# dylkot/cNMF

Measured on NVIDIA H100. Metric: NMF restarts/sec on NxG counts, K-sweep x100 seeds, 1/2/4/8 H100 vs sklearn CPU, higher is better.
Workload: dtype f32 (2-pass split-fp16 tensor-core products of group-normalised factors x exact integer counts, fp32 accumulate)

## Files before the change

### cnmf_b200/csrc/nmf_kernels.cu

```cuda
#include "nmf_kernels.cuh"

#include <cuda_fp16.h>

namespace cnmf {

namespace {

constexpr float EPSILON_F32 = 1.1920928955078125e-07f;

template <typename T>
__device__ __forceinline__ T block_sum(T v, T* smem ) {
  const int lane = threadIdx.x & 31, warp = threadIdx.x >> 5;
  v = warp_sum(v);
  __syncthreads();
  if (lane == 0) smem[warp] = v;
  __syncthreads();
  const int nw = (blockDim.x + 31) >> 5;
  T r = (threadIdx.x < nw) ? smem[threadIdx.x] : T(0);
  if (warp == 0) r = warp_sum(r);
  return r;
}

__global__ void split_tf32_kernel(const float* __restrict__ src, float* __restrict__ hi, float* __restrict__ lo,
                                  long long n4) {
// ... 227 lines not shown

template <int KP, int VEC>
__device__ __forceinline__ void load_items(const float* __restrict__ pF, const float* __restrict__ pN, int nsplit,
                                           long long sstride, int K, unsigned ld, int n_left,
                                           float2 (&fv)[KP][VecIO<VEC>::NP], float2 (&nv)[KP][VecIO<VEC>::NP]) {
  constexpr int NP = VecIO<VEC>::NP;
#pragma unroll
  for (int i = 0; i < KP; ++i) {
    if (i < K) {
      const unsigned off = (unsigned)i * ld;
      VecIO<VEC>::ld(pF + off, fv[i]);
      VecIO<VEC>::ld(pN + off, nv[i]);
    } else {
#pragma unroll
      for (int p = 0; p < NP; ++p) {
        fv[i][p] = make_float2(0.f, 0.f);
        nv[i][p] = make_float2(0.f, 0.f);
      }
    }
  }
  if (nsplit > 1) {
    for (int s = 1; s < nsplit; ++s) {
      const float* pS = pN + s * sstride;
#pragma unroll
      for (int i = 0; i < KP; ++i) {
        if (i < K) {
          float2 t[NP];
          VecIO<VEC>::ld(pS + (unsigned)i * ld, t);
#pragma unroll
          for (int p = 0; p < NP; ++p) nv[i][p] = add2(nv[i][p], t[p]);
        }
      }
    }
  }
  if (n_left < VEC) {
#pragma unroll
    for (int i = 0; i < KP; ++i)
#pragma unroll
      for (int p = 0; p < NP; ++p) {
        if (2 * p >= n_left) { nv[i][p].x = 0.f; fv[i][p].x = 0.f; }
        if (2 * p + 1 >= n_left) { nv[i][p].y = 0.f; fv[i][p].y = 0.f; }
      }
  }
}

template <int VEC>
__device__ __forceinline__ void store_items(float* pF, float* pH, float* pL, unsigned off,
                                            const float2 (&v)[VecIO<VEC>::NP], const float2 (&pscale)[VecIO<VEC>::NP]) {
  constexpr int NP = VecIO<VEC>::NP;
  VecIO<VEC>::st(pF + off, v);
  if (pH) {
    float2 h[NP], l[NP];
#pragma unroll
    for (int p = 0; p < NP; ++p) {
      const float2 sv = mul2(v[p], pscale[p]);
      h[p] = make_float2(to_tf32(sv.x), to_tf32(sv.y));
      const float2 rest = add2(sv, neg2(h[p]));
      l[p] = make_float2(to_tf32(rest.x), to_tf32(rest.y));
    }
    VecIO<VEC>::st(pH + off, h);
    VecIO<VEC>::st(pL + off, l);
  }
}

template <int KP> struct FusedGramCfg {
  static constexpr int WARPS = UPD_THREADS / 32;
  static constexpr int TPC = KP <= 4 ? 1 : (KP <= 8 ? 2 : 4);
  static constexpr int RB = KP / TPC;
  static constexpr int NG = WARPS / TPC;
  static constexpr int VALS = RB * KP;
  static constexpr int STRIDE = (VALS / 4) % 2 ? VALS : VALS + 4;
};

template <int KP, int TILE>
__device__ __forceinline__ void fused_gram_tile(float* tile, double* gsum) {
  using C = FusedGramCfg<KP>;
  const int lane = threadIdx.x & 31, warp = threadIdx.x >> 5;
  const int rb = warp % C::TPC, grp = warp / C::TPC;
  float2 acc[C::RB][KP];
#pragma unroll
  for (int a = 0; a < C::RB; ++a)
#pragma unroll
    for (int i = 0; i < KP; ++i) acc[a][i] = make_float2(0.f, 0.f);
  const float4* t4 = reinterpret_cast<const float4*>(tile);
  constexpr int QUADS = TILE / 4, ROW4 = TILE / 4;
#pragma unroll 1
  for (int q = grp * 32 + lane; q < QUADS; q += 32 * C::NG) {
    float4 v[KP], va[C::RB];
#pragma unroll
    for (int i = 0; i < KP; ++i) v[i] = t4[i * ROW4 + q];
#pragma unroll
    for (int a = 0; a < C::RB; ++a) va[a] = t4[(rb * C::RB + a) * ROW4 + q];
#pragma unroll
    for (int a = 0; a < C::RB; ++a)
#pragma unroll
      for (int i = 0; i < KP; ++i) {
        acc[a][i] = fma2(make_float2(va[a].x, va[a].y), make_float2(v[i].x, v[i].y), acc[a][i]);
        acc[a][i] = fma2(make_float2(va[a].z, va[a].w), make_float2(v[i].z, v[i].w), acc[a][i]);
      }
  }
  __syncthreads();
  float* scratch = tile + threadIdx.x * C::STRIDE;
#pragma unroll
  for (int a = 0; a < C::RB; ++a)
#pragma unroll
    for (int i4 = 0; i4 < KP / 4; ++i4) {
      float4 q;
      q.x = acc[a][4 * i4 + 0].x + acc[a][4 * i4 + 0].y;
      q.y = acc[a][4 * i4 + 1].x + acc[a][4 * i4 + 1].y;
      q.z = acc[a][4 * i4 + 2].x + acc[a][4 * i4 + 2].y;
      q.w = acc[a][4 * i4 + 3].x + acc[a][4 * i4 + 3].y;
      *reinterpret_cast<float4*>(scratch + a * KP + 4 * i4) = q;
    }
  __syncthreads();
  for (int e = threadIdx.x; e < KP * KP; e += UPD_THREADS) {
    const int row = e / KP, i = e % KP;
    const int erb = row / C::RB, a = row % C::RB;
    double sum = 0.0;
#pragma unroll
    for (int g = 0; g < C::NG; ++g) {
      const float* src = tile + (size_t)((erb + C::TPC * g) * 32) * C::STRIDE + a * KP + i;
#pragma unroll 8
      for (int l = 0; l < 32; ++l) sum += (double)src[l * C::STRIDE];
    }
    gsum[e] += sum;
  }
  __syncthreads();
}

struct SymGramMap {
  static __device__ __forceinline__ void owner(int bi, int bj, int& warp, int& slot) {
    const int id = bi * 4 + bj - (bi * (bi + 1)) / 2;
    warp = id / 3;
    slot = id % 3;
  }
};

template <int KP, int TILE, int W>
__device__ __forceinline__ void sym_gram_accumulate(const float* tile, float2 (&acc)[3][KP / 4][KP / 4]) {
  constexpr int RB = KP / 4;
  constexpr int NB = W == 3 ? 1 : 3;
  constexpr int BI[3] = {W == 0 ? 0 : (W == 1 ? 0 : (W == 2 ? 1 : 3)), W == 0 ? 0 : (W == 1 ? 1 : 2), W == 0 ? 0 : (W == 1 ? 1 : 2)};
  constexpr int BJ[3] = {W == 0 ? 0 : (W == 1 ? 3 : (W == 2 ? 3 : 3)), W == 0 ? 1 : (W == 1 ? 1 : 2), W == 0 ? 2 : (W == 1 ? 2 : 3)};
  const int lane = threadIdx.x & 31;
  const float4* t4 = reinterpret_cast<const float4*>(tile);
  constexpr int QUADS = TILE / 4, ROW4 = TILE / 4;
#pragma unroll 1
  for (int q = lane; q < QUADS; q += 32) {
    float4 v[4][RB];
#pragma unroll
    for (int blk = 0; blk < 4; ++blk) {
      bool used = false;
#pragma unroll
      for (int k = 0; k < NB; ++k) used = used || BI[k] == blk || BJ[k] == blk;
      if (used) {
#pragma unroll
        for (int a = 0; a < RB; ++a) v[blk][a] = t4[(blk * RB + a) * ROW4 + q];
      }
    }
#pragma unroll
    for (int k = 0; k < NB; ++k)
#pragma unroll
      for (int a = 0; a < RB; ++a)
#pragma unroll
        for (int b = 0; b < RB; ++b) {
          const float4 x = v[BI[k]][a], y = v[BJ[k]][b];
          acc[k][a][b] = fma2(make_float2(x.x, x.y), make_float2(y.x, y.y), acc[k][a][b]);
          acc[k][a][b] = fma2(make_float2(x.z, x.w), make_float2(y.z, y.w), acc[k][a][b]);
        }
  }
}

template <int KP> struct SymGramPlan {
  static constexpr int NUP = KP * (KP + 1) / 2;
  static constexpr int ROUNDS = (NUP + UPD_THREADS - 1) / UPD_THREADS;
};
constexpr int SYM_PLAN_WORDS = 3 * 2 * UPD_THREADS;

template <int KP>
__device__ __forceinline__ void sym_gram_plan(int* plan) {
  constexpr int RB = KP / 4;
  constexpr int STRIDE = 3 * RB * RB + 1;
  static_assert(SymGramPlan<KP>::ROUNDS <= 2, "plan buffer holds two rounds");
#pragma unroll
  for (int r = 0; r < SymGramPlan<KP>::ROUNDS; ++r) {
    const int t = threadIdx.x + r * UPD_THREADS;
    int row = 0, rem = t;
    while (row < KP - 1 && rem >= KP - row) { rem -= KP - row; ++row; }
    const int i = row + rem;
    int src = -1, e1 = 0, e2 = 0;
    if (t < SymGramPlan<KP>::NUP) {
      int w, slot;
      SymGramMap::owner(row / RB, i / RB, w, slot);
      src = (w * 32) * STRIDE + (slot * RB + row % RB) * RB + i % RB;
      e1 = row * KP + i;
      e2 = i * KP + row;
    }
    plan[(r * 3 + 0) * UPD_THREADS + threadIdx.x] = src;
    plan[(r * 3 + 1) * UPD_THREADS + threadIdx.x] = e1;
    plan[(r * 3 + 2) * UPD_THREADS + threadIdx.x] = e2;
  }
}

template <int KP, int TILE>
__device__ __forceinline__ void fused_gram_tile_sym(float* tile, double* gsum, const int* plan) {
  constexpr int RB = KP / 4;
  constexpr int STRIDE = 3 * RB * RB + 1;
  static_assert(UPD_THREADS == 128, "four warps share the ten blocks");
  static_assert(UPD_THREADS * STRIDE <= KP * TILE, "reduction scratch must fit in the tile it aliases");
  const int warp = threadIdx.x >> 5;
  float2 acc[3][RB][RB];
#pragma unroll
  for (int k = 0; k < 3; ++k)
#pragma unroll
    for (int a = 0; a < RB; ++a)
#pragma unroll
      for (int b = 0; b < RB; ++b) acc[k][a][b] = make_float2(0.f, 0.f);
  switch (warp) {
    case 0: sym_gram_accumulate<KP, TILE, 0>(tile, acc); break;
    case 1: sym_gram_accumulate<KP, TILE, 1>(tile, acc); break;
    case 2: sym_gram_accumulate<KP, TILE, 2>(tile, acc); break;
    default: sym_gram_accumulate<KP, TILE, 3>(tile, acc); break;
  }
  __syncthreads();
  float* scratch = tile + threadIdx.x * STRIDE;
#pragma unroll
  for (int k = 0; k < 3; ++k)
#pragma unroll
    for (int a = 0; a < RB; ++a)
#pragma unroll
      for (int b = 0; b < RB; ++b) scratch[(k * RB + a) * RB + b] = acc[k][a][b].x + acc[k][a][b].y;
  __syncthreads();
#pragma unroll
  for (int r = 0; r < SymGramPlan<KP>::ROUNDS; ++r) {
    const int so = plan[(r * 3 + 0) * UPD_THREADS + threadIdx.x];
    if (so >= 0) {
      const int e1 = plan[(r * 3 + 1) * UPD_THREADS + threadIdx.x], e2 = plan[(r * 3 + 2) * UPD_THREADS + threadIdx.x];
      const float* src = tile + so;
      double sum = 0.0;
#pragma unroll 8
      for (int l = 0; l < 32; ++l) sum += (double)src[l * STRIDE];
      gsum[e1] += sum;
      if (e2 != e1) gsum[e2] += sum;
    }
  }
  __syncthreads();
}

template <int TILE>
__device__ __forceinline__ void emit_tile_f16(const FactorView& f, const float* tile, int K, int o, int t0) {
  static_assert(TILE == 512, "one lane owns four 16-byte groups of a 512-column tile");
  const int lane = threadIdx.x & 31, warp = threadIdx.x >> 5;
  float4 ps[4];
#pragma unroll
  for (int j = 0; j < 4; ++j) {
    const int col = t0 + 4 * lane + 128 * j;
    ps[j] = make_float4(1.f, 1.f, 1.f, 1.f);
    if (f.piece_scale && col < f.ld) ps[j] = *reinterpret_cast<const float4*>(f.piece_scale + col);
  }
  const int group = t0 / TILE;
  for (int c = warp; c < K; c += UPD_THREADS / 32) {
    const float4* src = reinterpret_cast<const float4*>(tile + c * TILE);
    float2 v[4][2];
    float m = 0.f;
#pragma unroll
    for (int j = 0; j < 4; ++j) {
      const float4 q = src[lane + 32 * j];
      v[j][0] = mul2(make_float2(q.x, q.y), make_float2(ps[j].x, ps[j].y));
      v[j][1] = mul2(make_float2(q.z, q.w), make_float2(ps[j].z, ps[j].w));
      m = fmaxf(fmaxf(m, fmaxf(v[j][0].x, v[j][0].y)), fmaxf(v[j][1].x, v[j][1].y));
    }
#pragma unroll
    for (int s = 16; s > 0; s >>= 1) m = fmaxf(m, __shfl_xor_sync(0xffffffffu, m, s));
    const float sc = f16_group_scale(m);
    const float2 inv = bcast2(__uint_as_float(0x7f000000u - __float_as_uint(sc)));
    const long long rowoff = (long long)(o + c) * f.ld;
    if (lane == 0) f.tile_scale[(long long)(o + c) * f.n_ktiles + group] = sc;
    __half* ph = static_cast<__half*>(f.P_hi) + rowoff + t0 + 4 * lane;
    __half* pm = static_cast<__half*>(f.P_mid) + rowoff + t0 + 4 * lane;
    const int cols_left = f.ld - (t0 + 4 * lane);
#pragma unroll
    for (int j = 0; j < 4; ++j) {
      if (128 * j < cols_left) {
        const float2 x01 = mul2(v[j][0], inv), x23 = mul2(v[j][1], inv);
        const __half2 h01 = __float22half2_rn(x01), h23 = __float22half2_rn(x23);
        const float2 r01 = add2(x01, neg2(__half22float2(h01))), r23 = add2(x23, neg2(__half22float2(h23)));
        const __half2 m01 = __float22half2_rn(r01), m23 = __float22half2_rn(r23);
        uint2 oh, om;
        oh.x = *reinterpret_cast<const uint32_t*>(&h01); oh.y = *reinterpret_cast<const uint32_t*>(&h23);
        om.x = *reinterpret_cast<const uint32_t*>(&m01); om.y = *reinterpret_cast<const uint32_t*>(&m23);
        *reinterpret_cast<uint2*>(ph + 128 * j) = oh;
        *reinterpret_cast<uint2*>(pm + 128 * j) = om;
      }
    }
  }
}

__device__ __forceinline__ float4 lds128(unsigned addr) {
  float4 v;
  asm("ld.shared.v4.f32 {%0, %1, %2, %3}, [%4];" : "=f"(v.x), "=f"(v.y), "=f"(v.z), "=f"(v.w) : "r"(addr));
  return v;
}

template <int KP, int VEC, bool GRAM, bool RAGGED, bool SIMPLE>
__device__ __forceinline__ float2 mu_components(float* __restrict__ pFc, float* pH, float* pL, const float* __restrict__ pNc,
                                                int nsplit, long long sstride, unsigned ld, unsigned g_row, int K, float l1,
                                                float l2, int n_left, const float2 (&fv)[KP][VecIO<VEC>::NP],
                                                const float2 (&pscale)[VecIO<VEC>::NP], float* myF) {
  constexpr int NP = VecIO<VEC>::NP;
  constexpr int TILE = UPD_THREADS * VEC;
  float2 sacc = make_float2(0.f, 0.f);
  float2 nvn[NP], nvn2[NP];
  VecIO<VEC>::ld(pNc, nvn);
  VecIO<VEC>::ld(pNc + (1 < K ? ld : 0u), nvn2);
#pragma unroll 3
  for (int c = 0; c < K; ++c) {
    float2 den[NP];
#pragma unroll
    for (int i4 = 0; i4 < KP / 4; ++i4) {
      const float4 gq = lds128(g_row + 16 * i4);
#pragma unroll
      for (int p = 0; p < NP; ++p) {
        den[p] = i4 == 0 ? mul2(bcast2(gq.x), fv[0][p]) : fma2(bcast2(gq.x), fv[4 * i4 + 0][p], den[p]);
        den[p] = fma2(bcast2(gq.y), fv[4 * i4 + 1][p], den[p]);
        den[p] = fma2(bcast2(gq.z), fv[4 * i4 + 2][p], den[p]);
        den[p] = fma2(bcast2(gq.w), fv[4 * i4 + 3][p], den[p]);
      }
    }
    g_row += 4 * KP;
    float2 fvc[NP], nvc[NP], out[NP];
    VecIO<VEC>::ld(myF, fvc);
#pragma unroll
    for (int p = 0; p < NP; ++p) { nvc[p] = nvn[p]; nvn[p] = nvn2[p]; }
    VecIO<VEC>::ld(pNc + ((c + 2 < K) ? 2u * ld : 0u), nvn2);
    if constexpr (!SIMPLE) {
      for (int s = 1; s < nsplit; ++s) {
        float2 t[NP];
        VecIO<VEC>::ld(pNc + s * sstride, t);
#pragma unroll
        for (int p = 0; p < NP; ++p) nvc[p] = add2(nvc[p], t[p]);
      }
    }
    if constexpr (RAGGED) {
#pragma unroll
      for (int p = 0; p < NP; ++p) {
        if (2 * p >= n_left) nvc[p].x = 0.f;
        if (2 * p + 1 >= n_left) nvc[p].y = 0.f;
      }
    }
#pragma unroll
    for (int p = 0; p < NP; ++p) {
      float2 d = fma2(bcast2(l2), fvc[p], add2(den[p], bcast2(l1)));
      d.x = (d.x < FLT_MIN_NORMAL) ? EPSILON_F32 : d.x;
      d.y = (d.y < FLT_MIN_NORMAL) ? EPSILON_F32 : d.y;
      out[p] = mul2(fvc[p], div_nr2(nvc[p], d));
      sacc = fma2(nvc[p], out[p], sacc);
    }
    if constexpr (SIMPLE) {
      VecIO<VEC>::st(pFc, out);
    } else {
      store_items<VEC>(pFc, pH, pL, 0u, out, pscale);
      if (pH) { pH += ld; pL += ld; }
    }
    if constexpr (GRAM) VecIO<VEC>::st(myF, out);
    pFc += ld;
    pNc += ld;
    myF += TILE;
  }
  return sacc;
}

template <int KP, int VEC, bool GRAM, bool STREAMN>
__device__ __forceinline__ double mu_body(const FactorView& f, const float* __restrict__ NUM, int nsplit,
                                          long long sstride, const float* G, int K, int o, float l1, float l2,
                                          int col_begin, int col_end, float* tileF, float* tileN, double* gsum) {
  constexpr int NP = VecIO<VEC>::NP;
  constexpr int TILE = UPD_THREADS * VEC;
  const float4* G4 = reinterpret_cast<const float4*>(G);
  const unsigned g_addr = (unsigned)__cvta_generic_to_shared(G);
  const bool simple = nsplit == 1 && f.F_hi == nullptr;
  const unsigned ld = (unsigned)f.ld;
  float* const myF = tileF + VEC * threadIdx.x;
  float* const myN = tileN + VEC * threadIdx.x;
  double scal = 0.0;
  constexpr bool SYM = GRAM && VEC == 4 && (KP == 12 || KP == 16);
  __shared__ int gplan[SYM ? SYM_PLAN_WORDS : 1];
  if constexpr (SYM) sym_gram_plan<KP>(gplan);
#pragma unroll 1
  for (int t0 = col_begin; t0 < col_end; t0 += TILE) {
    const int col = t0 + VEC * threadIdx.x;
    if (col < col_end) {
      const long long e0 = (long long)o * f.ld + col;
      float* const pF = f.F + e0;
      float* const pH = f.F_hi ? f.F_hi + e0 : nullptr;
      float* const pL = f.F_hi ? f.F_lo + e0 : nullptr;
      float2 fv[KP][NP];
      const float* const pN = NUM + e0;
      const int n_left = f.n - col;
      if constexpr (STREAMN) {
#pragma unroll
        for (int i = 0; i < KP; ++i) {
          if (i < K) {
            VecIO<VEC>::ld(pF + (unsigned)i * ld, fv[i]);
          } else {
#pragma unroll
            for (int p = 0; p < NP; ++p) fv[i][p] = make_float2(0.f, 0.f);
          }
        }
        if (n_left < VEC) {
#pragma unroll
          for (int i = 0; i < KP; ++i)
#pragma unroll
            for (int p = 0; p < NP; ++p) {
              if (2 * p >= n_left) fv[i][p].x = 0.f;
              if (2 * p + 1 >= n_left) fv[i][p].y = 0.f;
            }
        }
#pragma unroll
        for (int i = 0; i < KP; ++i) VecIO<VEC>::st(myF + i * TILE, fv[i]);
      } else {
        float2 nv[KP][NP];
        load_items<KP, VEC>(pF, pN, nsplit, sstride, K, ld, n_left, fv, nv);
#pragma unroll
        for (int i = 0; i < KP; ++i) {
          VecIO<VEC>::st(myF + i * TILE, fv[i]);
          VecIO<VEC>::st(myN + i * TILE, nv[i]);
        }
      }
      float2 pscale[NP];
#pragma unroll
      for (int p = 0; p < NP; ++p) pscale[p] = make_float2(1.f, 1.f);
      if (f.piece_scale) VecIO<VEC>::ld(f.piece_scale + col, pscale);
      float2 sacc = make_float2(0.f, 0.f);
      if constexpr (STREAMN) {
        if (simple) {
          if (n_left >= VEC)
            sacc = mu_components<KP, VEC, GRAM, false, true>(pF, pH, pL, pN, 1, 0, ld, g_addr, K, l1, l2, n_left, fv, pscale, myF);
          else
            sacc = mu_components<KP, VEC, GRAM, true, true>(pF, pH, pL, pN, 1, 0, ld, g_addr, K, l1, l2, n_left, fv, pscale, myF);
        } else {
          if (n_left >= VEC)
            sacc = mu_components<KP, VEC, GRAM, false, false>(pF, pH, pL, pN, nsplit, sstride, ld, g_addr, K, l1, l2, n_left, fv,
                                                              pscale, myF);
          else
            sacc = mu_components<KP, VEC, GRAM, true, false>(pF, pH, pL, pN, nsplit, sstride, ld, g_addr, K, l1, l2, n_left, fv,
                                                             pscale, myF);
        }
      } else {
        unsigned off = 0;
#pragma unroll 1
        for (int c = 0; c < K; ++c, off += ld) {
          float2 den[NP];
#pragma unroll
          for (int i4 = 0; i4 < KP / 4; ++i4) {
            const float4 gq = G4[c * (KP / 4) + i4];
#pragma unroll
            for (int p = 0; p < NP; ++p) {
              den[p] = i4 == 0 ? mul2(bcast2(gq.x), fv[0][p]) : fma2(bcast2(gq.x), fv[4 * i4 + 0][p], den[p]);
              den[p] = fma2(bcast2(gq.y), fv[4 * i4 + 1][p], den[p]);
              den[p] = fma2(bcast2(gq.z), fv[4 * i4 + 2][p], den[p]);
              den[p] = fma2(bcast2(gq.w), fv[4 * i4 + 3][p], den[p]);
            }
          }
          float2 fvc[NP], nvc[NP], out[NP];
          VecIO<VEC>::ld(myF + c * TILE, fvc);
          VecIO<VEC>::ld(myN + c * TILE, nvc);
#pragma unroll
          for (int p = 0; p < NP; ++p) {
            const float2 d0 = fma2(bcast2(l2), fvc[p], add2(den[p], bcast2(l1)));
            float2 d = d0;
            d.x = (d.x < FLT_MIN_NORMAL) ? EPSILON_F32 : d.x;
            d.y = (d.y < FLT_MIN_NORMAL) ? EPSILON_F32 : d.y;
            out[p] = mul2(fvc[p], div_nr2(nvc[p], d));
            sacc = fma2(nvc[p], out[p], sacc);
          }
          store_items<VEC>(pF, pH, pL, off, out, pscale);
          if constexpr (GRAM) VecIO<VEC>::st(myF + c * TILE, out);
        }
      }
      scal += (double)(sacc.x + sacc.y);
    } else if constexpr (GRAM) {
      float2 z[NP];
#pragma unroll
      for (int p = 0; p < NP; ++p) z[p] = make_float2(0.f, 0.f);
#pragma unroll
      for (int c = 0; c < KP; ++c) VecIO<VEC>::st(myF + c * TILE, z);
    }
    if constexpr (GRAM) {
      __syncthreads();
      if constexpr (VEC == 4) {
        if (f.P_hi) emit_tile_f16<TILE>(f, tileF, K, o, t0);
      }
      if constexpr (SYM) fused_gram_tile_sym<KP, TILE>(tileF, gsum, gplan);
      else fused_gram_tile<KP, TILE>(tileF, gsum);
    }
  }
  return scal;
}

template <int KP, int VEC, bool GRAM>
__device__ __forceinline__ double cd_body(const FactorView& f, const float* __restrict__ NUM, int nsplit,
                                          long long sstride, const float* G, int K, int o, float l1,
                                          int col_begin, int col_end, float* tile, double* gsum) {
  constexpr int NP = VecIO<VEC>::NP;
  constexpr int TILE = UPD_THREADS * VEC;
  const volatile float4* Gv = reinterpret_cast<const volatile float4*>(G);
  const volatile float* Gs = G;
  const unsigned ld = (unsigned)f.ld;
  double scal = 0.0;
  constexpr bool SYM = GRAM && VEC == 4 && (KP == 12 || KP == 16);
  __shared__ int gplan[SYM ? SYM_PLAN_WORDS : 1];
  if constexpr (SYM) sym_gram_plan<KP>(gplan);
#pragma unroll 1
  for (int t0 = col_begin; t0 < col_end; t0 += TILE) {
    const int col = t0 + VEC * threadIdx.x;
    if (col < col_end) {
      const long long e0 = (long long)o * f.ld + col;
      float* const pF = f.F + e0;
      float* const pH = f.F_hi ? f.F_hi + e0 : nullptr;
      float* const pL = f.F_hi ? f.F_lo + e0 : nullptr;
      float2 fv[KP][NP], nv[KP][NP];
      load_items<KP, VEC>(pF, NUM + e0, nsplit, sstride, K, ld, f.n - col, fv, nv);
      float2 pscale[NP];
#pragma unroll
      for (int p = 0; p < NP; ++p) pscale[p] = make_float2(1.f, 1.f);
      if (f.piece_scale) VecIO<VEC>::ld(f.piece_scale + col, pscale);
      float2 sacc = make_float2(0.f, 0.f);
#pragma unroll
      for (int c = 0; c < KP; ++c) {
        float2 out[NP];
        if (c < K) {
          float2 g[NP];
#pragma unroll
          for (int p = 0; p < NP; ++p) g[p] = make_float2(l1 - nv[c][p].x, l1 - nv[c][p].y);
#pragma unroll
          for (int i4 = 0; i4 < KP / 4; ++i4) {
            const volatile float4& gq = Gv[c * (KP / 4) + i4];
            const float g0 = gq.x, g1 = gq.y, g2 = gq.z, g3 = gq.w;
#pragma unroll
            for (int p = 0; p < NP; ++p) {
              g[p] = fma2(bcast2(g0), fv[4 * i4 + 0][p], g[p]);
              g[p] = fma2(bcast2(g1), fv[4 * i4 + 1][p], g[p]);
              g[p] = fma2(bcast2(g2), fv[4 * i4 + 2][p], g[p]);
              g[p] = fma2(bcast2(g3), fv[4 * i4 + 3][p], g[p]);
            }
          }
          const float h = Gs[c * KP + c];
          const float hinv = Gs[KP * KP + c];
#pragma unroll
          for (int p = 0; p < NP; ++p) {
            const float pgx = (fv[c][p].x == 0.f) ? fminf(0.f, g[p].x) : g[p].x;
            const float pgy = (fv[c][p].y == 0.f) ? fminf(0.f, g[p].y) : g[p].y;
            sacc.x += fabsf(pgx);
            sacc.y += fabsf(pgy);
            if (h != 0.f) {
              float2 q = mul2(g[p], bcast2(hinv));
              const float2 rem = fma2(bcast2(-h), q, g[p]);
              q = fma2(bcast2(hinv), rem, q);
              fv[c][p].x = fmaxf(fv[c][p].x - q.x, 0.f);
              fv[c][p].y = fmaxf(fv[c][p].y - q.y, 0.f);
            }
            out[p] = fv[c][p];
          }
          store_items<VEC>(pF, pH, pL, (unsigned)c * ld, out, pscale);
        } else {
#pragma unroll
          for (int p = 0; p < NP; ++p) out[p] = make_float2(0.f, 0.f);
        }
        if constexpr (GRAM) VecIO<VEC>::st(tile + c * TILE + VEC * threadIdx.x, out);
      }
      scal += (double)(sacc.x + sacc.y);
    } else if constexpr (GRAM) {
      float2 z[NP];
#pragma unroll
      for (int p = 0; p < NP; ++p) z[p] = make_float2(0.f, 0.f);
#pragma unroll
      for (int c = 0; c < KP; ++c) VecIO<VEC>::st(tile + c * TILE + VEC * threadIdx.x, z);
    }
    if constexpr (GRAM) {
      __syncthreads();
      if constexpr (VEC == 4) {
        if (f.P_hi) emit_tile_f16<TILE>(f, tile, K, o, t0);
      }
      if constexpr (SYM) fused_gram_tile_sym<KP, TILE>(tile, gsum, gplan);
      else fused_gram_tile<KP, TILE>(tile, gsum);
    }
  }
  return scal;
}

#define CNMF_KP_SWITCH(K, KPMAX, CALL)                                            \
  switch (((K) + 3) / 4) {                                                        \
    case 1: { constexpr int KP = 4; CALL; } break;                                \
    case 2: { constexpr int KP = 8; CALL; } break;                                \
    case 3: { constexpr int KP = 12; CALL; } break;                               \
    case 4: { constexpr int KP = 16; CALL; } break;                               \
    case 5: if constexpr (KPMAX >= 20) { constexpr int KP = 20; CALL; } break;    \
    case 6: if constexpr (KPMAX >= 24) { constexpr int KP = 24; CALL; } break;    \
    case 7: if constexpr (KPMAX >= 28) { constexpr int KP = 28; CALL; } break;    \
    default: if constexpr (KPMAX >= 32) { constexpr int KP = 32; CALL; } break;   \
  }

template <int KPMAX, bool CD, bool GRAM, int MINB = (KPMAX == 32 ? 2 : 3), bool STREAMN = false>
__global__ void __launch_bounds__(UPD_THREADS, MINB)
update_kernel(FactorView f, const float* __restrict__ NUM, int nsplit, long long sstride,
              const double* __restrict__ gram_in, BatchMeta b, float l1, float l2, FusedOut out) {
  constexpr int VEC = KPMAX == 16 ? 4 : 2;
  const int slot = blockIdx.y;
  const int r = b.rid[slot];
  if (b.done[r]) return;
  const int K = b.k[slot], o = b.off[slot];
  const int KPr = ((K + 3) / 4) * 4;
  __shared__ __align__(16) float G[KPMAX * KPMAX + KPMAX];
  __shared__ double gsum[GRAM ? KPMAX * KPMAX : 1];
  __shared__ double red[32];
  __shared__ int s_last;
  extern __shared__ __align__(16) float tile[];
  load_gram_smem(G, gram_in, r, K, KPr, CD ? l2 : 0.f);
  if constexpr (GRAM)
    for (int e = threadIdx.x; e < KPr * KPr; e += UPD_THREADS) gsum[e] = 0.0;
  __syncthreads();
  if constexpr (CD) {
    if (threadIdx.x < KPr) {
      const float h = G[threadIdx.x * KPr + threadIdx.x];
      G[KPr * KPr + threadIdx.x] = (h != 0.f) ? rcp_nr(fmaxf(fabsf(h), FLT_MIN_NORMAL)) * (h < 0.f ? -1.f : 1.f) : 0.f;
    }
    __syncthreads();
  }
  const int col_begin = blockIdx.x * f.cpb;
  const int col_end = min(f.n, col_begin + f.cpb);
  const bool want_scal = out.scal_part != nullptr;
  double scal = 0.0;
  if constexpr (CD) {
    CNMF_KP_SWITCH(K, KPMAX, (scal = cd_body<KP, VEC, GRAM>(f, NUM, nsplit, sstride, G, K, o, l1, col_begin, col_end,
                                                             tile, gsum)));
  } else {
    float* tileN = tile + UPD_TILE_F_FLOATS;
    CNMF_KP_SWITCH(K, KPMAX, (scal = mu_body<KP, VEC, GRAM, STREAMN>(f, NUM, nsplit, sstride, G, K, o, l1, l2, col_begin, col_end,
                                                                      tile, tileN, gsum)));
  }
  const int chunks = gridDim.x;
  if (want_scal) {
    scal = block_sum(scal, red);
    if (threadIdx.x == 0) out.scal_part[(long long)slot * chunks + blockIdx.x] = scal;
  }
  const int stride = b.kp * b.kp;
  if constexpr (GRAM) {
    double* part = out.gram_part + ((long long)slot * chunks + blockIdx.x) * stride;
    for (int e = threadIdx.x; e < KPr * KPr; e += UPD_THREADS) part[e] = gsum[e];
  }
  if (!GRAM && !want_scal) return;
  __threadfence();
  __syncthreads();
  if (threadIdx.x == 0) s_last = (atomicAdd(&out.counter[r], 1) == chunks - 1);
  __syncthreads();
  if (!s_last) return;
  __threadfence();
  if constexpr (GRAM) {
    const double* part = out.gram_part + (long long)slot * chunks * stride;
    for (int e = threadIdx.x; e < KPr * KPr; e += UPD_THREADS) {
      double a = 0.0;
#pragma unroll 4
      for (int ch = 0; ch < chunks; ++ch) a += __ldcg(part + (long long)ch * stride + e);
      out.gram[(long long)r * KMAX * KMAX + (e / KPr) * KMAX + (e % KPr)] = a;
    }
  }
  if (want_scal && threadIdx.x < 32) {
    double a = 0.0;
    for (int ch = threadIdx.x; ch < chunks; ch += 32) a += __ldcg(out.scal_part + (long long)slot * chunks + ch);
    a = warp_sum(a);
    if (threadIdx.x == 0) out.scal[r] = a;
  }
  if (threadIdx.x == 0) out.counter[r] = 0;
}

__global__ void __launch_bounds__(UPD_THREADS)
cross_kernel(FactorView f, const float* __restrict__ NUM, int nsplit, long long sstride, BatchMeta b,
             double* __restrict__ cross_partial) {
  const int slot = blockIdx.y;
  const int r = b.rid[slot];
  if (b.done[r]) return;
  const int K = b.k[slot], o = b.off[slot];
  __shared__ double red[32];
  const int col_begin = blockIdx.x * f.cpb;
  const int col_end = min(f.n, col_begin + f.cpb);
  double cross = 0.0;
  for (int col = col_begin + threadIdx.x; col < col_end; col += UPD_THREADS) {
    for (int c = 0; c < K; ++c) {
      const long long e = (long long)(o + c) * f.ld + col;
      float num = NUM[e];
      for (int s = 1; s < nsplit; ++s) num += NUM[s * sstride + e];
      cross += (double)num * (double)f.F[e];
    }
  }
  cross = block_sum(cross, red);
  if (threadIdx.x == 0) cross_partial[(long long)r * gridDim.x + blockIdx.x] = cross;
}

template <int KP, int BT>
struct GramCfg {
  static constexpr int TPC = KP <= 8 ? 1 : (KP <= 16 ? 2 : (KP <= 24 ? 4 : 8));
  static constexpr int RB = (KP + TPC - 1) / TPC;
  static constexpr int VEC = KP <= 12 ? 4 : 2;
  static constexpr int COLS_PER_ITER = (BT / TPC) * VEC;
  static constexpr int WARPS = BT / 32;
};

template <int VEC> struct VecLoad;
template <> struct VecLoad<4> {
  static __device__ __forceinline__ void ld(const float* p, float (&v)[4]) {
    const float4 q = *reinterpret_cast<const float4*>(p);
    v[0] = q.x; v[1] = q.y; v[2] = q.z; v[3] = q.w;
  }
};
template <> struct VecLoad<2> {
  static __device__ __forceinline__ void ld(const float* p, float (&v)[2]) {
    const float2 q = *reinterpret_cast<const float2*>(p);
    v[0] = q.x; v[1] = q.y;
  }
};

template <int KP, int BT>
__device__ __forceinline__ void gram_body(const FactorView& f, int K, int o, int col_begin, int col_end,
                                          double* part , double* __restrict__ out) {
  using C = GramCfg<KP, BT>;
  const int rb = threadIdx.x % C::TPC;
  const int cl = threadIdx.x / C::TPC;
  float acc[C::RB][KP];
#pragma unroll
  for (int a = 0; a < C::RB; ++a)
#pragma unroll
    for (int i = 0; i < KP; ++i) acc[a][i] = 0.f;
  const float* __restrict__ Fp = f.F;
  for (int col = col_begin + cl * C::VEC; col < col_end; col += C::COLS_PER_ITER) {
    float fv[KP][C::VEC];
#pragma unroll
    for (int i = 0; i < KP; ++i) {
      if (i < K) {
        VecLoad<C::VEC>::ld(Fp + (long long)(o + i) * f.ld + col, fv[i]);
      } else {
#pragma unroll
        for (int u = 0; u < C::VEC; ++u) fv[i][u] = 0.f;
      }
    }
#pragma unroll
    for (int u = 0; u < C::VEC; ++u) {
#pragma unroll
      for (int a = 0; a < C::RB; ++a) {
        float fa = 0.f;
#pragma unroll
        for (int t = 0; t < C::TPC; ++t)
          if (t == rb && t * C::RB + a < KP) fa = fv[t * C::RB + a < KP ? t * C::RB + a : 0][u];
#pragma unroll
        for (int i = 0; i < KP; ++i) acc[a][i] = fmaf(fa, fv[i][u], acc[a][i]);
      }
    }
  }
  const int lane = threadIdx.x & 31, warp = threadIdx.x >> 5;
#pragma unroll
  for (int a = 0; a < C::RB; ++a) {
    double v[KP];
#pragma unroll
    for (int i = 0; i < KP; ++i) v[i] = (double)acc[a][i];
#pragma unroll
    for (int sh = 16; sh >= C::TPC; sh >>= 1)
#pragma unroll
      for (int i = 0; i < KP; ++i) v[i] += __shfl_xor_sync(0xffffffffu, v[i], sh);
    __syncthreads();
    if (lane < C::TPC) {
#pragma unroll
      for (int i = 0; i < KP; ++i) part[(warp * 8 + lane) * 32 + i] = v[i];
    }
    __syncthreads();
    for (int t = threadIdx.x; t < C::TPC * KP; t += BT) {
      const int rbb = t / KP, i = t % KP;
      const int row = rbb * C::RB + a;
      if (row < KP) {
        double sum = 0.0;
#pragma unroll
        for (int w = 0; w < C::WARPS; ++w) sum += part[(w * 8 + rbb) * 32 + i];
        out[row * KP + i] = sum;
      }
    }
  }
}

template <int KPMAX, int BT>
__global__ void __launch_bounds__(BT)
gram_partial_kernel(FactorView f, BatchMeta b, double* __restrict__ gram_partial) {
  const int slot = blockIdx.y;
  const int r = b.rid[slot];
  if (b.done[r]) return;
  const int K = b.k[slot], o = b.off[slot];
  __shared__ double part[(BT / 32) * 8 * 32];
  const int col_begin = blockIdx.x * f.gcpb;
  const int col_end = min(f.n, col_begin + f.gcpb);
  double* out = gram_partial + ((long long)r * gridDim.x + blockIdx.x) * (KPMAX * KPMAX);
  CNMF_KP_SWITCH(K, KPMAX, (gram_body<KP, BT>(f, K, o, col_begin, col_end, part, out)));
}

__global__ void finalize_kernel(const double* __restrict__ gram_partial, double* __restrict__ gram,
                                const double* __restrict__ scal_partial, double* __restrict__ scal, int chunks,
                                BatchMeta b) {
  const int r = b.rid[blockIdx.x];
  if (b.done[r]) return;
  if (gram_partial) {
    const int K = b.k[blockIdx.x];
    const int KP = ((K + 3) / 4) * 4;
    const int stride = b.kp * b.kp;
    for (int e = threadIdx.x; e < KP * KP; e += blockDim.x) {
      double a = 0.0;
      for (int ch = 0; ch < chunks; ++ch) a += gram_partial[((long long)r * chunks + ch) * stride + e];
      const int c = e / KP, i = e % KP;
      gram[(long long)r * KMAX * KMAX + c * KMAX + i] = a;
    }
  }
  if (scal_partial && threadIdx.x == 0) {
    double a = 0.0;
    for (int ch = 0; ch < chunks; ++ch) a += scal_partial[(long long)r * chunks + ch];
    scal[r] = a;
  }
}

__global__ void mu_check_kernel(ConvState st, const double* __restrict__ cross, const double* __restrict__ gramA,
                                const double* __restrict__ gramB, double normX2, BatchMeta b, int it, double tol,
                                int max_iter) {
  const int slot = (blockIdx.x * blockDim.x + threadIdx.x) >> 5, lane = threadIdx.x & 31;
  if (slot >= b.R) return;
  const int r = b.rid[slot];
  if (st.done[r]) return;
  const int K = b.k[slot];
  double dot = 0.0;
  for (int e = lane; e < K * K; e += 32) {
    const int c = e / K, i = e % K;
    dot += gramA[(long long)r * KMAX * KMAX + c * KMAX + i] * gramB[(long long)r * KMAX * KMAX + c * KMAX + i];
  }
  dot = warp_sum(dot);
  if (lane != 0) return;
  const double err = sqrt(fmax(normX2 - 2.0 * cross[r] + dot, 0.0));
  st.last[r] = err;
  if (it == 0) {
    st.err0[r] = err;
    st.prev[r] = err;
    return;
  }
  if ((st.prev[r] - err) / st.err0[r] < tol) {
    st.done[r] = 1;
    st.n_iter[r] = it;
  } else {
    st.prev[r] = err;
    if (it >= max_iter) {
      st.done[r] = 1;
      st.n_iter[r] = it;
    }
  }
}

__global__ void cd_check_kernel(ConvState st, const double* __restrict__ violA, const double* __restrict__ violB,
                                BatchMeta b, int it, double tol, int max_iter) {
  const int slot = blockIdx.x * blockDim.x + threadIdx.x;
  if (slot >= b.R) return;
  const int r = b.rid[slot];
  if (st.done[r]) return;
  const double viol = violA[r] + (violB ? violB[r] : 0.0);
  st.last[r] = viol;
  if (it == 1) st.err0[r] = viol;
  const double v0 = st.err0[r];
  if (v0 == 0.0 || viol / v0 <= tol || it >= max_iter) {
    st.done[r] = 1;
    st.n_iter[r] = it;
  }
}

__global__ void gather_rows_kernel(const float* __restrict__ src, const int* __restrict__ src_off,
                                   float* __restrict__ dst, const int* __restrict__ dst_off,
                                   const int* __restrict__ k, int ld) {
  const int r = blockIdx.x / KMAX, c = blockIdx.x % KMAX;
  if (c >= k[r]) return;
  const float4* s = reinterpret_cast<const float4*>(src + (long long)(src_off[r] + c) * ld);
  float4* d = reinterpret_cast<float4*>(dst + (long long)(dst_off[r] + c) * ld);
  for (int i = threadIdx.x; i < ld / 4; i += blockDim.x) d[i] = s[i];
}

}

int launch_split_tf32(const float* src, float* hi, float* lo, long long n_elems, cudaStream_t s) {
  CNMF_REQUIRE(n_elems % 4 == 0, "split_tf32: element count must be a multiple of 4");
  const long long n4 = n_elems / 4;
  if (n4 == 0) return 0;
  const int blocks = (int)((n4 + 255) / 256 < NUM_SMS * 16 ? (n4 + 255) / 256 : NUM_SMS * 16);
  split_tf32_kernel<<<blocks, 256, 0, s>>>(src, hi, lo, n4);
  CNMF_CUDA_CHECK(cudaGetLastError());
  return 0;
}

int launch_split_scaled(const float* src, float* hi, float* lo, int rows, int ld, const float* col_scale, cudaStream_t s) {
  CNMF_REQUIRE(ld % 4 == 0, "split_scaled: ld must be a multiple of 4");
  const long long n4 = (long long)rows * (ld / 4);
  if (n4 == 0) return 0;
  const int blocks = (int)((n4 + 255) / 256 < NUM_SMS * 16 ? (n4 + 255) / 256 : NUM_SMS * 16);
  split_scaled_kernel<<<blocks, 256, 0, s>>>(src, hi, lo, rows, ld, col_scale);
  CNMF_CUDA_CHECK(cudaGetLastError());
  return 0;
}

int launch_emit_f16(const float* F, int rows, int n, int ld, const float* pscale, void* hi, void* mid, float* tile_scale,
                    int n_ktiles, cudaStream_t s) {
  CNMF_REQUIRE(ld % 8 == 0 && (long long)n_ktiles * 512 >= ld, "emit_f16: bad ld / n_ktiles");
  if (rows <= 0) return 0;
  emit_f16_kernel<4><<<rows, 256, 0, s>>>(F, n, ld, pscale, static_cast<__half*>(hi), static_cast<__half*>(mid), tile_scale,
                                          n_ktiles);
  CNMF_CUDA_CHECK(cudaGetLastError());
  return 0;
}

int launch_to_half(const float* src, void* dst, long long n_elems, cudaStream_t s) {
  CNMF_REQUIRE(n_elems % 4 == 0, "to_half: element count must be a multiple of 4");
  const long long n4 = n_elems / 4;
  if (n4 == 0) return 0;
  const int blocks = (int)((n4 + 255) / 256 < NUM_SMS * 16 ? (n4 + 255) / 256 : NUM_SMS * 16);
  to_half_kernel<<<blocks, 256, 0, s>>>(src, static_cast<__half*>(dst), n4);
  CNMF_CUDA_CHECK(cudaGetLastError());
  return 0;
}

int launch_min_positive(const float* X, int rows, int cols, int ld, float* col_min, float* row_min, cudaStream_t s) {
  CNMF_CUDA_CHECK(cudaMemsetAsync(col_min, 0x7f, sizeof(float) * cols, s));
  CNMF_CUDA_CHECK(cudaMemsetAsync(row_min, 0x7f, sizeof(float) * rows, s));
  dim3 grid((cols + 255) / 256, (rows + 63) / 64);
  CNMF_REQUIRE(grid.y <= 65535, "min_positive: too many rows for one launch");
  min_positive_kernel<<<grid, 256, 0, s>>>(X, rows, cols, ld, reinterpret_cast<int*>(col_min), reinterpret_cast<int*>(row_min));
  CNMF_CUDA_CHECK(cudaGetLastError());
  return 0;
}

int launch_check_scaled_int(const float* X, int rows, int cols, int ld, const float* row_scale, const float* col_scale,
                            int* n_bad, cudaStream_t s) {
  check_scaled_int_kernel<<<NUM_SMS * 8, 256, 0, s>>>(X, rows, cols, ld, row_scale, col_scale, n_bad);
  CNMF_CUDA_CHECK(cudaGetLastError());
  return 0;
}

int launch_build_counts(const float* X, int rows, int cols, int ld, const float* row_scale, const float* col_scale,
                        float* C, cudaStream_t s) {
  build_counts_kernel<<<NUM_SMS * 8, 256, 0, s>>>(X, rows, cols, ld, row_scale, col_scale, C);
  CNMF_CUDA_CHECK(cudaGetLastError());
  return 0;
}

int launch_fix_scale(float* v, int n, int n_pad, cudaStream_t s) {
  fix_scale_kernel<<<(n_pad + 255) / 256, 256, 0, s>>>(v, n, n_pad);
  CNMF_CUDA_CHECK(cudaGetLastError());
  return 0;
}

int launch_transpose(const float* src, int rows, int cols, int ld_src, float* dst, float* dst_hi, float* dst_lo,
                     int ld_dst, cudaStream_t s) {
  dim3 grid((cols + 31) / 32, (rows + 31) / 32), block(32, 8);
  CNMF_REQUIRE(grid.y <= 65535, "transpose: too many rows for one launch");
  transpose_kernel<<<grid, block, 0, s>>>(src, rows, cols, ld_src, dst, dst_hi, dst_lo, ld_dst);
  CNMF_CUDA_CHECK(cudaGetLastError());
  return 0;
}

int launch_matrix_sums(const float* X, int rows, int cols, int ld, double* out2, double* scratch, int scratch_len,
                       cudaStream_t s) {
  int blocks = NUM_SMS * 8;
  if (2 * blocks > scratch_len) blocks = scratch_len / 2;
  CNMF_REQUIRE(blocks >= 1, "matrix_sums: scratch too small");
  sums_partial_kernel<<<blocks, 256, 0, s>>>(X, rows, cols, ld, scratch);
  sums_final_kernel<<<1, 256, 0, s>>>(scratch, blocks, out2);
  CNMF_CUDA_CHECK(cudaGetLastError());
  return 0;
}

#define CNMF_DISPATCH_KPMAX(kp, CALL)                               \
  switch (kp) {                                                      \
    case 16: { constexpr int KPMAX = 16; CALL; } break;              \
    case 32: { constexpr int KPMAX = 32; CALL; } break;              \
    default: set_last_error("kp must be 16 or 32"); return -1;       \
  }

template <int KPMAX, bool CD, bool GRAM, int MINB, bool STREAMN>
static int launch_update_inst(dim3 grid, const FactorView& f, const float* NUM, int nsplit, long long sstride,
                              const double* gram_in, const BatchMeta& b, float l1, float l2, const FusedOut& out,
                              cudaStream_t s) {
  const size_t smem = sizeof(float) * (CD ? (GRAM ? (size_t)UPD_TILE_F_FLOATS : 0)
                                          : (size_t)UPD_TILE_F_FLOATS + (STREAMN ? 0 : UPD_TILE_N_FLOATS));
  static bool attr_set[64] = {};
  int dev = 0;
  CNMF_CUDA_CHECK(cudaGetDevice(&dev));
  if (smem > 0 && (dev < 0 || dev >= 64 || !attr_set[dev])) {
    CNMF_CUDA_CHECK(cudaFuncSetAttribute(update_kernel<KPMAX, CD, GRAM, MINB, STREAMN>,
                                         cudaFuncAttributeMaxDynamicSharedMemorySize, (int)smem));
    if (dev >= 0 && dev < 64) attr_set[dev] = true;
  }
  update_kernel<KPMAX, CD, GRAM, MINB, STREAMN><<<grid, UPD_THREADS, smem, s>>>(f, NUM, nsplit, sstride, gram_in, b, l1, l2, out);
  CNMF_CUDA_CHECK(cudaGetLastError());
  return 0;
}

template <int KPMAX, bool CD, bool GRAM>
static int launch_update_variant(dim3 grid, const FactorView& f, const float* NUM, int nsplit, long long sstride,
                                 const double* gram_in, const BatchMeta& b, float l1, float l2, const FusedOut& out,
                                 cudaStream_t s) {
  if constexpr (KPMAX == 16 && !CD && GRAM)
    return launch_update_inst<KPMAX, CD, GRAM, 4, true>(grid, f, NUM, nsplit, sstride, gram_in, b, l1, l2, out, s);
  else
    return launch_update_inst<KPMAX, CD, GRAM, (KPMAX == 32 ? 2 : 3), false>(grid, f, NUM, nsplit, sstride, gram_in, b, l1, l2, out, s);
}

template <bool CD>
static int launch_update(const FactorView& f, const float* NUM, int nsplit, long long sstride, const double* gram_in,
                         const BatchMeta& b, float l1, float l2, const FusedOut& out, cudaStream_t s) {
  CNMF_REQUIRE(f.cpb % upd_tile_cols(b.kp) == 0, "update: cpb must be a multiple of the update tile");
  CNMF_REQUIRE(f.ld % 4 == 0, "update: ld must be a multiple of 4");
  static_assert(16 * UPD_THREADS * 4 == UPD_TILE_N_FLOATS && 32 * UPD_THREADS * 2 == UPD_TILE_N_FLOATS, "tile sizes");
  dim3 grid(col_chunks(f), b.R);
  if (b.kp == 16) {
    if (out.gram_part) return launch_update_variant<16, CD, true>(grid, f, NUM, nsplit, sstride, gram_in, b, l1, l2, out, s);
    return launch_update_variant<16, CD, false>(grid, f, NUM, nsplit, sstride, gram_in, b, l1, l2, out, s);
  }
  if (b.kp == 32) {
    CNMF_REQUIRE(out.gram_part == nullptr, "update: the fused Gram exists for kp == 16 batches only");
    return launch_update_variant<32, CD, false>(grid, f, NUM, nsplit, sstride, gram_in, b, l1, l2, out, s);
  }
  set_last_error("kp must be 16 or 32");
  return -1;
}

int launch_mu_update(const FactorView& f, const float* NUM, int nsplit, long long sstride, const double* gram_in,
                     const BatchMeta& b, float l1, float l2, const FusedOut& out, cudaStream_t s) {
  return launch_update<false>(f, NUM, nsplit, sstride, gram_in, b, l1, l2, out, s);
}

int launch_cd_update(const FactorView& f, const float* NUM, int nsplit, long long sstride, const double* gram_in,
                     const BatchMeta& b, float l1, float l2, const FusedOut& out, cudaStream_t s) {
  return launch_update<true>(f, NUM, nsplit, sstride, gram_in, b, l1, l2, out, s);
}

int launch_cross(const FactorView& f, const float* NUM, int nsplit, long long sstride, const BatchMeta& b,
                 double* cross_partial, cudaStream_t s) {
  dim3 grid(col_chunks(f), b.R);
  cross_kernel<<<grid, UPD_THREADS, 0, s>>>(f, NUM, nsplit, sstride, b, cross_partial);
  CNMF_CUDA_CHECK(cudaGetLastError());
  return 0;
}

int launch_gram_partial(const FactorView& f, const BatchMeta& b, double* gram_partial, cudaStream_t s, bool one_warp_blocks) {
  dim3 grid(gram_chunks(f), b.R);
  if (one_warp_blocks) {
    CNMF_DISPATCH_KPMAX(b.kp, (gram_partial_kernel<KPMAX, 32><<<grid, 32, 0, s>>>(f, b, gram_partial)));
  } else {
    CNMF_DISPATCH_KPMAX(b.kp, (gram_partial_kernel<KPMAX, 256><<<grid, 256, 0, s>>>(f, b, gram_partial)));
  }
  CNMF_CUDA_CHECK(cudaGetLastError());
  return 0;
}

int launch_finalize(const double* gram_partial, double* gram, const double* scal_partial, double* scal, int chunks,
                    const BatchMeta& b, cudaStream_t s) {
  finalize_kernel<<<b.R, 256, 0, s>>>(gram_partial, gram, scal_partial, scal, chunks, b);
  CNMF_CUDA_CHECK(cudaGetLastError());
  return 0;
}

int launch_mu_check(const ConvState& st, const double* cross, const double* gramA, const double* gramB, double normX2,
                    const BatchMeta& b, int it, double tol, int max_iter, cudaStream_t s) {
  mu_check_kernel<<<(b.R + 3) / 4, 128, 0, s>>>(st, cross, gramA, gramB, normX2, b, it, tol, max_iter);
  CNMF_CUDA_CHECK(cudaGetLastError());
  return 0;
}

int launch_cd_check(const ConvState& st, const double* violA, const double* violB, const BatchMeta& b, int it,
                    double tol, int max_iter, cudaStream_t s) {
  cd_check_kernel<<<(b.R + 127) / 128, 128, 0, s>>>(st, violA, violB, b, it, tol, max_iter);
  CNMF_CUDA_CHECK(cudaGetLastError());
  return 0;
}

int launch_gather_rows(const float* src, const int* src_off, float* dst, const int* dst_off, const int* k, int R,
                       int ld, cudaStream_t s) {
  if (R == 0) return 0;
  gather_rows_kernel<<<R * KMAX, 128, 0, s>>>(src, src_off, dst, dst_off, k, ld);
  CNMF_CUDA_CHECK(cudaGetLastError());
  return 0;
}

}
```

Measured before the change: 526.3.

## Prefetch factor and numerator tiles with TMA bulk copies and mbarriers in MU update

Adds a pipelined variant of the fused multiplicative-update W path. Thread 0 issues cp.async.bulk copies of the next 512-column tile of the factor rows and numerator rows into shared-memory stages, and mbarriers signal when each stage has landed, so global loads overlap with the update math and the Gram accumulation. It is selected when nsplit==1, there is no hi/lo split, the f16 P output exists and the chunk is large enough. In exchange it uses more shared memory and drops launch bounds to 2 blocks per SM, which lowers occupancy. There are also extra block-wide syncs per tile.

Result: faster. 531.8 (median of 6 runs) (+1.0%).

```diff
diff --git a/cnmf_b200/csrc/nmf_kernels.cu b/cnmf_b200/csrc/nmf_kernels.cu
--- a/cnmf_b200/csrc/nmf_kernels.cu
+++ b/cnmf_b200/csrc/nmf_kernels.cu
@@ -553,17 +553,18 @@
   return v;
 }
 
-template <int KP, int VEC, bool GRAM, bool RAGGED, bool SIMPLE>
+template <int KP, int VEC, bool GRAM, bool RAGGED, bool SIMPLE, int NLD = 0>
 __device__ __forceinline__ float2 mu_components(float* __restrict__ pFc, float* pH, float* pL, const float* __restrict__ pNc,
                                                 int nsplit, long long sstride, unsigned ld, unsigned g_row, int K, float l1,
                                                 float l2, int n_left, const float2 (&fv)[KP][VecIO<VEC>::NP],
                                                 const float2 (&pscale)[VecIO<VEC>::NP], float* myF) {
   constexpr int NP = VecIO<VEC>::NP;
   constexpr int TILE = UPD_THREADS * VEC;
+  const unsigned nld = NLD ? (unsigned)NLD : ld;
   float2 sacc = make_float2(0.f, 0.f);
   float2 nvn[NP], nvn2[NP];
   VecIO<VEC>::ld(pNc, nvn);
-  VecIO<VEC>::ld(pNc + (1 < K ? ld : 0u), nvn2);
+  VecIO<VEC>::ld(pNc + (1 < K ? nld : 0u), nvn2);
 #pragma unroll 3
   for (int c = 0; c < K; ++c) {
     float2 den[NP];
@@ -583,7 +584,7 @@
     VecIO<VEC>::ld(myF, fvc);
 #pragma unroll
     for (int p = 0; p < NP; ++p) { nvc[p] = nvn[p]; nvn[p] = nvn2[p]; }
-    VecIO<VEC>::ld(pNc + ((c + 2 < K) ? 2u * ld : 0u), nvn2);
+    VecIO<VEC>::ld(pNc + ((c + 2 < K) ? 2u * nld : 0u), nvn2);
     if constexpr (!SIMPLE) {
       for (int s = 1; s < nsplit; ++s) {
         float2 t[NP];
@@ -615,7 +616,7 @@
     }
     if constexpr (GRAM) VecIO<VEC>::st(myF, out);
     pFc += ld;
-    pNc += ld;
+    pNc += nld;
     myF += TILE;
   }
   return sacc;
@@ -749,6 +750,114 @@
   return scal;
 }
 
+constexpr int PIPE_STAGE_FLOATS = 16 * 512;
+
+__device__ __forceinline__ void pipe_bar_init(uint32_t bar) {
+  asm volatile("mbarrier.init.shared::cta.b64 [%0], 1;" ::"r"(bar) : "memory");
+}
+__device__ __forceinline__ void pipe_bar_wait(uint32_t bar, uint32_t parity) {
+  uint32_t ok = 0;
+  while (!ok) {
+    asm volatile(
+        "{\n\t.reg .pred p;\n\t"
+        "mbarrier.try_wait.parity.shared::cta.b64 p, [%1], %2;\n\t"
+        "selp.u32 %0, 1, 0, p;\n\t}"
+        : "=r"(ok)
+        : "r"(bar), "r"(parity)
+        : "memory");
+  }
+}
+__device__ __forceinline__ void pipe_load_rows(uint32_t stage, const float* src, int K, unsigned ld, int t0, uint32_t bar) {
+  const uint32_t bytes = 4u * (uint32_t)min(512, (int)ld - t0);
+  asm volatile("fence.proxy.async.shared::cta;" ::: "memory");
+  asm volatile("mbarrier.arrive.expect_tx.shared::cta.b64 _, [%0], %1;" ::"r"(bar), "r"(bytes * (uint32_t)K) : "memory");
+  for (int i = 0; i < K; ++i)
+    asm volatile("cp.async.bulk.shared::cluster.global.mbarrier::complete_tx::bytes [%0], [%1], %2, [%3];"
+                 ::"r"(stage + 2048u * i), "l"(src + (size_t)i * ld + t0), "r"(bytes), "r"(bar)
+                 : "memory");
+}
+
+template <int KP>
+__device__ __forceinline__ double mu_body_pipe(const FactorView& f, const float* __restrict__ NUM, const float* G, int K,
+                                               int o, float l1, float l2, int col_begin, int col_end, float* tileF,
+                                               const float* sF, const float* sN, uint32_t barF, uint32_t barN,
+                                               double* gsum) {
+  constexpr int VEC = 4, NP = VecIO<VEC>::NP, TILE = UPD_THREADS * VEC;
+  static_assert(TILE == 512 && KP <= 16, "stage rows are one 512-column tile of at most 16 components");
+  const unsigned g_addr = (unsigned)__cvta_generic_to_shared(G);
+  const unsigned ld = (unsigned)f.ld;
+  const uint32_t stF = (uint32_t)__cvta_generic_to_shared(sF), stN = (uint32_t)__cvta_generic_to_shared(sN);
+  const float* const rowF = f.F + (long long)o * f.ld;
+  const float* const rowN = NUM + (long long)o * f.ld;
+  float* const myF = tileF + VEC * threadIdx.x;
+  double scal = 0.0;
+  constexpr bool SYM = KP == 12 || KP == 16;
+  __shared__ int gplan[SYM ? SYM_PLAN_WORDS : 1];
+  if constexpr (SYM) sym_gram_plan<KP>(gplan);
+  uint32_t parity = 0;
+#pragma unroll 1
+  for (int t0 = col_begin; t0 < col_end; t0 += TILE, parity ^= 1u) {
+    const int col = t0 + VEC * threadIdx.x;
+    const bool active = col < col_end;
+    const int n_left = f.n - col;
+    const int t1 = t0 + TILE;
+    float2 fv[KP][NP];
+    pipe_bar_wait(barF, parity);
+    if (active) {
+#pragma unroll
+      for (int i = 0; i < KP; ++i) {
+        if (i < K) {
+          VecIO<VEC>::ld(sF + i * TILE + VEC * threadIdx.x, fv[i]);
+        } else {
+#pragma unroll
+          for (int p = 0; p < NP; ++p) fv[i][p] = make_float2(0.f, 0.f);
+        }
+      }
+      if (n_left < VEC) {
+#pragma unroll
+        for (int i = 0; i < KP; ++i)
+#pragma unroll
+          for (int p = 0; p < NP; ++p) {
+            if (2 * p >= n_left) fv[i][p].x = 0.f;
+            if (2 * p + 1 >= n_left) fv[i][p].y = 0.f;
+          }
+      }
+    }
+    __syncthreads();
+    if (threadIdx.x == 0 && t1 < col_end) pipe_load_rows(stF, rowF, K, ld, t1, barF);
+    if (active) {
+#pragma unroll
+      for (int i = 0; i < KP; ++i) VecIO<VEC>::st(myF + i * TILE, fv[i]);
+      float2 pscale[NP];
+#pragma unroll
+      for (int p = 0; p < NP; ++p) pscale[p] = make_float2(1.f, 1.f);
+      float* const pF = f.F + (long long)o * f.ld + col;
+      const float* const pN = sN + VEC * threadIdx.x;
+      pipe_bar_wait(barN, parity);
+      float2 sacc;
+      if (n_left >= VEC)
+        sacc = mu_components<KP, VEC, true, false, true, TILE>(pF, nullptr, nullptr, pN, 1, 0, ld, g_addr, K, l1, l2, n_left,
+                                                               fv, pscale, myF);
+      else
+        sacc = mu_components<KP, VEC, true, true, true, TILE>(pF, nullptr, nullptr, pN, 1, 0, ld, g_addr, K, l1, l2, n_left,
+                                                              fv, pscale, myF);
+      scal += (double)(sacc.x + sacc.y);
+    } else {
+      float2 z[NP];
+#pragma unroll
+      for (int p = 0; p < NP; ++p) z[p] = make_float2(0.f, 0.f);
+#pragma unroll
+      for (int c = 0; c < KP; ++c) VecIO<VEC>::st(myF + c * TILE, z);
+    }
+    __syncthreads();
+    if (threadIdx.x == 0 && t1 < col_end) pipe_load_rows(stN, rowN, K, ld, t1, barN);
+    emit_tile_f16<TILE>(f, tileF, K, o, t0);
+    if constexpr (SYM) fused_gram_tile_sym<KP, TILE>(tileF, gsum, gplan);
+    else fused_gram_tile<KP, TILE>(tileF, gsum);
+  }
+  return scal;
+}
+
 template <int KP, int VEC, bool GRAM>
 __device__ __forceinline__ double cd_body(const FactorView& f, const float* __restrict__ NUM, int nsplit,
                                           long long sstride, const float* G, int K, int o, float l1,
@@ -852,10 +961,11 @@
     default: if constexpr (KPMAX >= 32) { constexpr int KP = 32; CALL; } break;   \
   }
 
-template <int KPMAX, bool CD, bool GRAM, int MINB = (KPMAX == 32 ? 2 : 3), bool STREAMN = false>
+template <int KPMAX, bool CD, bool GRAM, int MINB = (KPMAX == 32 ? 2 : 3), bool STREAMN = false, bool PIPE = false>
 __global__ void __launch_bounds__(UPD_THREADS, MINB)
 update_kernel(FactorView f, const float* __restrict__ NUM, int nsplit, long long sstride,
               const double* __restrict__ gram_in, BatchMeta b, float l1, float l2, FusedOut out) {
+  static_assert(!PIPE || (KPMAX == 16 && !CD && GRAM), "the bulk-copy pipeline is the W half of the f16x2 MU path");
   constexpr int VEC = KPMAX == 16 ? 4 : 2;
   const int slot = blockIdx.y;
   const int r = b.rid[slot];
@@ -866,7 +976,23 @@
   __shared__ double gsum[GRAM ? KPMAX * KPMAX : 1];
   __shared__ double red[32];
   __shared__ int s_last;
+  __shared__ uint64_t pipe_bar[PIPE ? 2 : 1];
   extern __shared__ __align__(16) float tile[];
+  const int col_begin = blockIdx.x * f.cpb;
+  const int col_end = min(f.n, col_begin + f.cpb);
+  if constexpr (PIPE) {
+    if (threadIdx.x == 0) {
+      const uint32_t bF = (uint32_t)__cvta_generic_to_shared(&pipe_bar[0]);
+      const uint32_t bN = (uint32_t)__cvta_generic_to_shared(&pipe_bar[1]);
+      pipe_bar_init(bF);
+      pipe_bar_init(bN);
+      asm volatile("fence.mbarrier_init.release.cluster;" ::: "memory");
+      pipe_load_rows((uint32_t)__cvta_generic_to_shared(tile + UPD_TILE_F_FLOATS), f.F + (long long)o * f.ld, K,
+                     (unsigned)f.ld, col_begin, bF);
+      pipe_load_rows((uint32_t)__cvta_generic_to_shared(tile + UPD_TILE_F_FLOATS + PIPE_STAGE_FLOATS),
+                     NUM + (long long)o * f.ld, K, (unsigned)f.ld, col_begin, bN);
+    }
+  }
   load_gram_smem(G, gram_in, r, K, KPr, CD ? l2 : 0.f);
   if constexpr (GRAM)
     for (int e = threadIdx.x; e < KPr * KPr; e += UPD_THREADS) gsum[e] = 0.0;
@@ -878,13 +1004,17 @@
     }
     __syncthreads();
   }
-  const int col_begin = blockIdx.x * f.cpb;
-  const int col_end = min(f.n, col_begin + f.cpb);
   const bool want_scal = out.scal_part != nullptr;
   double scal = 0.0;
   if constexpr (CD) {
     CNMF_KP_SWITCH(K, KPMAX, (scal = cd_body<KP, VEC, GRAM>(f, NUM, nsplit, sstride, G, K, o, l1, col_begin, col_end,
                                                              tile, gsum)));
+  } else if constexpr (PIPE) {
+    const float* sF = tile + UPD_TILE_F_FLOATS;
+    const uint32_t bF = (uint32_t)__cvta_generic_to_shared(&pipe_bar[0]);
+    const uint32_t bN = (uint32_t)__cvta_generic_to_shared(&pipe_bar[1]);
+    CNMF_KP_SWITCH(K, KPMAX, (scal = mu_body_pipe<KP>(f, NUM, G, K, o, l1, l2, col_begin, col_end, tile, sF,
+                                                      sF + PIPE_STAGE_FLOATS, bF, bN, gsum)));
   } else {
     float* tileN = tile + UPD_TILE_F_FLOATS;
     CNMF_KP_SWITCH(K, KPMAX, (scal = mu_body<KP, VEC, GRAM, STREAMN>(f, NUM, nsplit, sstride, G, K, o, l1, l2, col_begin, col_end,
@@ -1232,21 +1362,23 @@
     default: set_last_error("kp must be 16 or 32"); return -1;       \
   }
 
-template <int KPMAX, bool CD, bool GRAM, int MINB, bool STREAMN>
+template <int KPMAX, bool CD, bool GRAM, int MINB, bool STREAMN, bool PIPE = false>
 static int launch_update_inst(dim3 grid, const FactorView& f, const float* NUM, int nsplit, long long sstride,
                               const double* gram_in, const BatchMeta& b, float l1, float l2, const FusedOut& out,
                               cudaStream_t s) {
   const size_t smem = sizeof(float) * (CD ? (GRAM ? (size_t)UPD_TILE_F_FLOATS : 0)
-                                          : (size_t)UPD_TILE_F_FLOATS + (STREAMN ? 0 : UPD_TILE_N_FLOATS));
+                                          : (size_t)UPD_TILE_F_FLOATS + (PIPE ? 2 * PIPE_STAGE_FLOATS
+                                                                              : (STREAMN ? 0 : UPD_TILE_N_FLOATS)));
   static bool attr_set[64] = {};
   int dev = 0;
   CNMF_CUDA_CHECK(cudaGetDevice(&dev));
   if (smem > 0 && (dev < 0 || dev >= 64 || !attr_set[dev])) {
-    CNMF_CUDA_CHECK(cudaFuncSetAttribute(update_kernel<KPMAX, CD, GRAM, MINB, STREAMN>,
+    CNMF_CUDA_CHECK(cudaFuncSetAttribute(update_kernel<KPMAX, CD, GRAM, MINB, STREAMN, PIPE>,
                                          cudaFuncAttributeMaxDynamicSharedMemorySize, (int)smem));
     if (dev >= 0 && dev < 64) attr_set[dev] = true;
   }
-  update_kernel<KPMAX, CD, GRAM, MINB, STREAMN><<<grid, UPD_THREADS, smem, s>>>(f, NUM, nsplit, sstride, gram_in, b, l1, l2, out);
+  update_kernel<KPMAX, CD, GRAM, MINB, STREAMN, PIPE><<<grid, UPD_THREADS, smem, s>>>(f, NUM, nsplit, sstride, gram_in, b, l1,
+                                                                                      l2, out);
   CNMF_CUDA_CHECK(cudaGetLastError());
   return 0;
 }
@@ -1255,9 +1387,11 @@
 static int launch_update_variant(dim3 grid, const FactorView& f, const float* NUM, int nsplit, long long sstride,
                                  const double* gram_in, const BatchMeta& b, float l1, float l2, const FusedOut& out,
                                  cudaStream_t s) {
-  if constexpr (KPMAX == 16 && !CD && GRAM)
+  if constexpr (KPMAX == 16 && !CD && GRAM) {
+    if (nsplit == 1 && f.F_hi == nullptr && f.P_hi != nullptr && f.cpb >= 4 * UPD_THREADS * 4)
+      return launch_update_inst<KPMAX, CD, GRAM, 2, true, true>(grid, f, NUM, nsplit, sstride, gram_in, b, l1, l2, out, s);
     return launch_update_inst<KPMAX, CD, GRAM, 4, true>(grid, f, NUM, nsplit, sstride, gram_in, b, l1, l2, out, s);
-  else
+  } else
     return launch_update_inst<KPMAX, CD, GRAM, (KPMAX == 32 ? 2 : 3), false>(grid, f, NUM, nsplit, sstride, gram_in, b, l1, l2, out, s);
 }
 
```
